# iwa-shi/CRDR

Hardware: AMD Instinct MI355X
Metric: stage-3 training img/s at 256x256 (higher is better)
Workload: dtype fp32; 1 GPU; config/crdr_stage_3.yaml -b 16: full GAN step (G + 5x CLIC21GVAE D + LPIPS-Alex, random-init weights), rate index cycled 0..4; global_batch=16, crop=256, parallelism=dp1

## Files before the change

crdr_amd/csrc/igemm.hip:

```cpp
#include <algorithm>
#include <type_traits>

#include "algo_id.hpp"
#include "igemm_kernel.hpp"
#include "wino.hpp"

namespace crdr {

extern template __global__ void igemm_kernel<4, 1, 1, 1, false, 0, false>(const IgemmArgs, const IgemmTaps, const IgemmGroup);
extern template __global__ void igemm_kernel<4, 1, 1, 2, false, 0, false>(const IgemmArgs, const IgemmTaps, const IgemmGroup);
extern template __global__ void igemm_kernel<4, 1, 1, 3, false, 0, false>(const IgemmArgs, const IgemmTaps, const IgemmGroup);
extern template __global__ void igemm_kernel<4, 1, 1, 4, false, 0, false>(const IgemmArgs, const IgemmTaps, const IgemmGroup);
extern template __global__ void igemm_kernel<4, 1, 1, 5, false, 0, false>(const IgemmArgs, const IgemmTaps, const IgemmGroup);
extern template __global__ void igemm_kernel<4, 1, 1, 6, false, 0, false>(const IgemmArgs, const IgemmTaps, const IgemmGroup);
extern template __global__ void igemm_kernel<4, 1, 1, 7, false, 0, false>(const IgemmArgs, const IgemmTaps, const IgemmGroup);
extern template __global__ void igemm_kernel<4, 1, 2, 2, false, 0, false>(const IgemmArgs, const IgemmTaps, const IgemmGroup);
extern template __global__ void igemm_kernel<4, 1, 2, 3, false, 0, false>(const IgemmArgs, const IgemmTaps, const IgemmGroup);
extern template __global__ void igemm_kernel<4, 1, 2, 4, false, 0, false>(const IgemmArgs, const IgemmTaps, const IgemmGroup);
extern template __global__ void igemm_kernel<2, 2, 2, 2, false, 0, false>(const IgemmArgs, const IgemmTaps, const IgemmGroup);
extern template __global__ void igemm_kernel<2, 2, 1, 1, false, 0, false>(const IgemmArgs, const IgemmTaps, const IgemmGroup);
extern template __global__ void igemm_kernel<2, 2, 1, 2, false, 0, false>(const IgemmArgs, const IgemmTaps, const IgemmGroup);
extern template __global__ void igemm_kernel<2, 2, 1, 3, false, 0, false>(const IgemmArgs, const IgemmTaps, const IgemmGroup);
extern template __global__ void igemm_kernel<2, 2, 1, 4, false, 0, false>(const IgemmArgs, const IgemmTaps, const IgemmGroup);
extern template __global__ void igemm_kernel<1, 4, 1, 1, false, 0, false>(const IgemmArgs, const IgemmTaps, const IgemmGroup);
extern template __global__ void igemm_kernel<1, 4, 1, 2, false, 0, false>(const IgemmArgs, const IgemmTaps, const IgemmGroup);
extern template __global__ void igemm_kernel<4, 2, 1, 1, false, 0, false>(const IgemmArgs, const IgemmTaps, const IgemmGroup);
extern template __global__ void igemm_kernel<4, 2, 1, 2, false, 0, false>(const IgemmArgs, const IgemmTaps, const IgemmGroup);
extern template __global__ void igemm_kernel<4, 2, 1, 3, false, 0, false>(const IgemmArgs, const IgemmTaps, const IgemmGroup);
extern template __global__ void igemm_kernel<4, 2, 2, 1, false, 0, false>(const IgemmArgs, const IgemmTaps, const IgemmGroup);
extern template __global__ void igemm_kernel<4, 2, 2, 2, false, 0, false>(const IgemmArgs, const IgemmTaps, const IgemmGroup);
extern template __global__ void igemm_kernel<2, 4, 1, 1, false, 0, false>(const IgemmArgs, const IgemmTaps, const IgemmGroup);
extern template __global__ void igemm_kernel<2, 4, 2, 1, false, 0, false>(const IgemmArgs, const IgemmTaps, const IgemmGroup);
extern template __global__ void igemm_kernel<2, 4, 1, 2, false, 0, false>(const IgemmArgs, const IgemmTaps, const IgemmGroup);
extern template __global__ void igemm_kernel<2, 2, 2, 1, false, 0, false>(const IgemmArgs, const IgemmTaps, const IgemmGroup);
extern template __global__ void igemm_kernel<2, 2, 2, 3, false, 0, false>(const IgemmArgs, const IgemmTaps, const IgemmGroup);
extern template __global__ void igemm_kernel<4, 1, 1, 1, true, 0, false>(const IgemmArgs, const IgemmTaps, const IgemmGroup);
extern template __global__ void igemm_kernel<4, 1, 1, 2, true, 0, false>(const IgemmArgs, const IgemmTaps, const IgemmGroup);
extern template __global__ void igemm_kernel<4, 1, 2, 2, true, 0, false>(const IgemmArgs, const IgemmTaps, const IgemmGroup);
extern template __global__ void igemm_kernel<2, 2, 2, 2, true, 0, false>(const IgemmArgs, const IgemmTaps, const IgemmGroup);
extern template __global__ void igemm_kernel<4, 2, 1, 1, true, 0, false>(const IgemmArgs, const IgemmTaps, const IgemmGroup);
extern template __global__ void igemm_kernel<4, 2, 1, 2, true, 0, false>(const IgemmArgs, const IgemmTaps, const IgemmGroup);
extern template __global__ void igemm_kernel<4, 2, 2, 1, true, 0, false>(const IgemmArgs, const IgemmTaps, const IgemmGroup);
extern template __global__ void igemm_kernel<4, 2, 2, 2, true, 0, false>(const IgemmArgs, const IgemmTaps, const IgemmGroup);
extern template __global__ void igemm_kernel<2, 4, 2, 1, true, 0, false>(const IgemmArgs, const IgemmTaps, const IgemmGroup);
extern template __global__ void igemm_kernel<4, 1, 1, 1, false, 3, false>(const IgemmArgs, const IgemmTaps, const IgemmGroup);
extern template __global__ void igemm_kernel<4, 1, 1, 2, false, 3, false>(const IgemmArgs, const IgemmTaps, const IgemmGroup);
extern template __global__ void igemm_kernel<4, 1, 1, 3, false, 3, false>(const IgemmArgs, const IgemmTaps, const IgemmGroup);
extern template __global__ void igemm_kernel<4, 1, 1, 4, false, 3, false>(const IgemmArgs, const IgemmTaps, const IgemmGroup);
extern template __global__ void igemm_kernel<4, 1, 1, 5, false, 3, false>(const IgemmArgs, const IgemmTaps, const IgemmGroup);
extern template __global__ void igemm_kernel<4, 1, 1, 6, false, 3, false>(const IgemmArgs, const IgemmTaps, const IgemmGroup);
extern template __global__ void igemm_kernel<4, 1, 1, 7, false, 3, false>(const IgemmArgs, const IgemmTaps, const IgemmGroup);
extern template __global__ void igemm_kernel<4, 1, 2, 2, false, 3, false>(const IgemmArgs, const IgemmTaps, const IgemmGroup);
extern template __global__ void igemm_kernel<4, 1, 2, 3, false, 3, false>(const IgemmArgs, const IgemmTaps, const IgemmGroup);
extern template __global__ void igemm_kernel<4, 1, 2, 4, false, 3, false>(const IgemmArgs, const IgemmTaps, const IgemmGroup);
extern template __global__ void igemm_kernel<2, 2, 2, 2, false, 3, false>(const IgemmArgs, const IgemmTaps, const IgemmGroup);
extern template __global__ void igemm_kernel<2, 2, 1, 1, false, 3, false>(const IgemmArgs, const IgemmTaps, const IgemmGroup);
extern template __global__ void igemm_kernel<2, 2, 1, 2, false, 3, false>(const IgemmArgs, const IgemmTaps, const IgemmGroup);
extern template __global__ void igemm_kernel<2, 2, 1, 3, false, 3, false>(const IgemmArgs, const IgemmTaps, const IgemmGroup);
extern template __global__ void igemm_kernel<2, 2, 1, 4, false, 3, false>(const IgemmArgs, const IgemmTaps, const IgemmGroup);
extern template __global__ void igemm_kernel<1, 4, 1, 1, false, 3, false>(const IgemmArgs, const IgemmTaps, const IgemmGroup);
extern template __global__ void igemm_kernel<1, 4, 1, 2, false, 3, false>(const IgemmArgs, const IgemmTaps, const IgemmGroup);
extern template __global__ void igemm_kernel<4, 2, 1, 1, false, 3, false>(const IgemmArgs, const IgemmTaps, const IgemmGroup);
extern template __global__ void igemm_kernel<4, 2, 1, 2, false, 3, false>(const IgemmArgs, const IgemmTaps, const IgemmGroup);
extern template __global__ void igemm_kernel<4, 2, 1, 3, false, 3, false>(const IgemmArgs, const IgemmTaps, const IgemmGroup);
extern template __global__ void igemm_kernel<4, 2, 2, 1, false, 3, false>(const IgemmArgs, const IgemmTaps, const IgemmGroup);
extern template __global__ void igemm_kernel<4, 2, 2, 2, false, 3, false>(const IgemmArgs, const IgemmTaps, const IgemmGroup);
extern template __global__ void igemm_kernel<2, 4, 1, 1, false, 3, false>(const IgemmArgs, const IgemmTaps, const IgemmGroup);
extern template __global__ void igemm_kernel<2, 4, 2, 1, false, 3, false>(const IgemmArgs, const IgemmTaps, const IgemmGroup);
extern template __global__ void igemm_kernel<2, 4, 1, 2, false, 3, false>(const IgemmArgs, const IgemmTaps, const IgemmGroup);
extern template __global__ void igemm_kernel<2, 2, 2, 1, false, 3, false>(const IgemmArgs, const IgemmTaps, const IgemmGroup);
extern template __global__ void igemm_kernel<2, 2, 2, 3, false, 3, false>(const IgemmArgs, const IgemmTaps, const IgemmGroup);
extern template __global__ void igemm_kernel<4, 1, 1, 2, false, 6, false>(const IgemmArgs, const IgemmTaps, const IgemmGroup);
extern template __global__ void igemm_kernel<4, 1, 1, 4, false, 6, false>(const IgemmArgs, const IgemmTaps, const IgemmGroup);
extern template __global__ void igemm_kernel<2, 2, 2, 2, false, 6, false>(const IgemmArgs, const IgemmTaps, const IgemmGroup);
extern template __global__ void igemm_kernel<2, 2, 1, 1, false, 6, false>(const IgemmArgs, const IgemmTaps, const IgemmGroup);
extern template __global__ void igemm_kernel<2, 2, 1, 2, false, 6, false>(const IgemmArgs, const IgemmTaps, const IgemmGroup);
extern template __global__ void igemm_kernel<2, 2, 1, 3, false, 6, false>(const IgemmArgs, const IgemmTaps, const IgemmGroup);
extern template __global__ void igemm_kernel<4, 2, 1, 2, false, 6, false>(const IgemmArgs, const IgemmTaps, const IgemmGroup);
extern template __global__ void igemm_kernel<2, 4, 2, 1, false, 6, false>(const IgemmArgs, const IgemmTaps, const IgemmGroup);
extern template __global__ void igemm_kernel<2, 2, 2, 1, false, 6, false>(const IgemmArgs, const IgemmTaps, const IgemmGroup);
extern template __global__ void igemm_kernel<4, 1, 1, 1, false, 0, true>(const IgemmArgs, const IgemmTaps, const IgemmGroup);
extern template __global__ void igemm_kernel<4, 1, 1, 2, false, 0, true>(const IgemmArgs, const IgemmTaps, const IgemmGroup);
extern template __global__ void igemm_kernel<4, 1, 1, 3, false, 0, true>(const IgemmArgs, const IgemmTaps, const IgemmGroup);
extern template __global__ void igemm_kernel<4, 1, 1, 4, false, 0, true>(const IgemmArgs, const IgemmTaps, const IgemmGroup);
extern template __global__ void igemm_kernel<4, 1, 1, 5, false, 0, true>(const IgemmArgs, const IgemmTaps, const IgemmGroup);
extern template __global__ void igemm_kernel<4, 1, 1, 6, false, 0, true>(const IgemmArgs, const IgemmTaps, const IgemmGroup);
extern template __global__ void igemm_kernel<4, 1, 1, 7, false, 0, true>(const IgemmArgs, const IgemmTaps, const IgemmGroup);
extern template __global__ void igemm_kernel<4, 1, 2, 2, false, 0, true>(const IgemmArgs, const IgemmTaps, const IgemmGroup);
extern template __global__ void igemm_kernel<4, 1, 2, 3, false, 0, true>(const IgemmArgs, const IgemmTaps, const IgemmGroup);
extern template __global__ void igemm_kernel<4, 1, 2, 4, false, 0, true>(const IgemmArgs, const IgemmTaps, const IgemmGroup);
extern template __global__ void igemm_kernel<2, 2, 2, 2, false, 0, true>(const IgemmArgs, const IgemmTaps, const IgemmGroup);
extern template __global__ void igemm_kernel<2, 2, 1, 1, false, 0, true>(const IgemmArgs, const IgemmTaps, const IgemmGroup);
extern template __global__ void igemm_kernel<2, 2, 1, 2, false, 0, true>(const IgemmArgs, const IgemmTaps, const IgemmGroup);
extern template __global__ void igemm_kernel<2, 2, 1, 3, false, 0, true>(const IgemmArgs, const IgemmTaps, const IgemmGroup);
extern template __global__ void igemm_kernel<2, 2, 1, 4, false, 0, true>(const IgemmArgs, const IgemmTaps, const IgemmGroup);
extern template __global__ void igemm_kernel<1, 4, 1, 1, false, 0, true>(const IgemmArgs, const IgemmTaps, const IgemmGroup);
extern template __global__ void igemm_kernel<1, 4, 1, 2, false, 0, true>(const IgemmArgs, const IgemmTaps, const IgemmGroup);
extern template __global__ void igemm_kernel<4, 2, 1, 1, false, 0, true>(const IgemmArgs, const IgemmTaps, const IgemmGroup);
extern template __global__ void igemm_kernel<4, 2, 1, 2, false, 0, true>(const IgemmArgs, const IgemmTaps, const IgemmGroup);
extern template __global__ void igemm_kernel<4, 2, 1, 3, false, 0, true>(const IgemmArgs, const IgemmTaps, const IgemmGroup);
extern template __global__ void igemm_kernel<4, 2, 2, 1, false, 0, true>(const IgemmArgs, const IgemmTaps, const IgemmGroup);
extern template __global__ void igemm_kernel<4, 2, 2, 2, false, 0, true>(const IgemmArgs, const IgemmTaps, const IgemmGroup);
extern template __global__ void igemm_kernel<2, 4, 1, 1, false, 0, true>(const IgemmArgs, const IgemmTaps, const IgemmGroup);
extern template __global__ void igemm_kernel<2, 4, 2, 1, false, 0, true>(const IgemmArgs, const IgemmTaps, const IgemmGroup);
extern template __global__ void igemm_kernel<2, 4, 1, 2, false, 0, true>(const IgemmArgs, const IgemmTaps, const IgemmGroup);
extern template __global__ void igemm_kernel<2, 2, 2, 1, false, 0, true>(const IgemmArgs, const IgemmTaps, const IgemmGroup);
extern template __global__ void igemm_kernel<2, 2, 2, 3, false, 0, true>(const IgemmArgs, const IgemmTaps, const IgemmGroup);

using IgemmKern = void (*)(const IgemmArgs, const IgemmTaps, const IgemmGroup);
enum TileForm {
  kPlain,
  kTapMajor,
  kBf3,
  kFast,
  kBf6,
  kNumTileForms
};
struct TileCfg {
  int wm, wn, mb, nb;
  IgemmKern kern[kNumTileForms];
};
static constexpr size_t cfg_lds(int wm, int wn, int mb, int nb, int prec) {
  const size_t BM = 32 * wm * mb, BN = 32 * wn * nb;
  const size_t staging = igemm_staging_floats((int)BM, (int)BN, prec);
  const size_t epi = (size_t)wm * wn * 32 * 32 * (nb < 4 ? nb : 4) + (size_t)wm * 2 * BN;
  const size_t sv_off = ((staging > epi ? staging : epi) + 3) & ~(size_t)3;
  return (sv_off + (size_t)4 * BN + 4) * sizeof(float);
}
template <int a, int b, int c, int d, bool FITS = igemm_bf6_ok(a, b, c, d) && (cfg_lds(a, b, c, d, 6) <= 160 * 1024)>
struct Bf6Kern { static constexpr IgemmKern fn = igemm_kernel<a, b, c, d, false, 6>; };
template <int a, int b, int c, int d>
struct Bf6Kern<a, b, c, d, false> { static constexpr IgemmKern fn = nullptr; };
#define CFG(a, b, c, d) {a, b, c, d, {igemm_kernel<a, b, c, d, false, 0>, nullptr, igemm_kernel<a, b, c, d, false, 3>, igemm_kernel<a, b, c, d, false, 0, true>, Bf6Kern<a, b, c, d>::fn}}
#define CFGS(a, b, c, d) {a, b, c, d, {igemm_kernel<a, b, c, d, false, 0>, igemm_kernel<a, b, c, d, true, 0>, igemm_kernel<a, b, c, d, false, 3>, igemm_kernel<a, b, c, d, false, 0, true>, Bf6Kern<a, b, c, d>::fn}}
static const TileCfg kCfgs[] = {
    CFGS(4, 1, 1, 1), CFGS(4, 1, 1, 2), CFG(4, 1, 1, 3), CFG(4, 1, 1, 4), CFG(4, 1, 1, 5), CFG(4, 1, 1, 6),
    CFG(4, 1, 1, 7),
    CFGS(4, 1, 2, 2), CFG(4, 1, 2, 3), CFG(4, 1, 2, 4),
    CFGS(2, 2, 2, 2),
    CFG(2, 2, 1, 1),
    CFG(2, 2, 1, 2),
    CFG(2, 2, 1, 3),
    CFG(2, 2, 1, 4),
    CFG(1, 4, 1, 1),
    CFG(1, 4, 1, 2),
    CFGS(4, 2, 1, 1),
    CFGS(4, 2, 1, 2),
    CFG(4, 2, 1, 3),
    CFGS(4, 2, 2, 1),
    CFGS(4, 2, 2, 2),
    CFG(2, 4, 1, 1),
    CFGS(2, 4, 2, 1),
    CFG(2, 4, 1, 2),
    CFG(2, 2, 2, 1),
    CFG(2, 2, 2, 3),
};
#undef CFG
#undef CFGS
static const int kNumCfgs = sizeof(kCfgs) / sizeof(kCfgs[0]);

struct Plan {
  IgemmArgs a;
  IgemmTaps t;
  int cfg;
  int stream;
  WinoKernel wino;
  StreamArgs sa;
  dim3 grid;
  size_t lds;
  size_t ws_bytes;
};

static bool splitk_ok(long long tiles, int M, int ws_ld, int ns) {
  return tiles <= CRDR_CONV_TICKETS && (long long)ns * M * ws_ld * 4 < (1ll << 31) - (1 << 24);
}

static int floordiv(int a, int b) {
  int q = a / b, r = a % b;
  return (r != 0 && ((r < 0) != (b < 0))) ? q - 1 : q;
}

static const float kCfgTflops[] = {107, 120, 122, 120, 105, 99, 94, 90, 101, 106, 102, 116, 123, 120, 107, 109, 111, 115, 126, 121,
                                   111, 116, 119, 127, 114, 119, 108};
static_assert(sizeof(kCfgTflops) / sizeof(kCfgTflops[0]) == sizeof(kCfgs) / sizeof(kCfgs[0]), "one figure per configuration");

static void fill_taps(const crdr_conv_desc* d, IgemmArgs& a, IgemmTaps& tp) {
  auto pack_tap = [](int dh, int dw, int widx) { return (dh & 0xff) | ((dw & 0xff) << 8) | (widx << 16); };
  const int S = d->stride, P = d->pad;
  int nt = 0;
  if (!d->transposed) {
    a.nphase = 1; a.GH = d->OH; a.GW = d->OW; a.so = 1; a.si = S;
    tp.poh[0] = 0; tp.pow[0] = 0; tp.tap_begin[0] = 0;
    for (int r = 0; r < d->kh; ++r)
      for (int s = 0; s < d->kw; ++s) {
        tp.packed[nt++] = pack_tap(r - P, s - P, r * d->kw + s);
      }
    tp.tap_begin[1] = (short)nt;
  } else {
    a.nphase = S * S; a.GH = cdiv(d->OH, S); a.GW = cdiv(d->OW, S); a.so = S; a.si = 1;
    int ph = 0;
    for (int py = 0; py < S; ++py)
      for (int px = 0; px < S; ++px, ++ph) {
        tp.poh[ph] = (int8_t)py; tp.pow[ph] = (int8_t)px; tp.tap_begin[ph] = (short)nt;
        for (int r = 0; r < d->kh; ++r) {
          if (((py + P - r) % S + S) % S) continue;
          for (int s = 0; s < d->kw; ++s) {
            if (((px + P - s) % S + S) % S) continue;
            tp.packed[nt++] = pack_tap(floordiv(py + P - r, S), floordiv(px + P - s, S), r * d->kw + s);
          }
        }
      }
    tp.tap_begin[ph] = (short)nt;
  }
}

static int plan_geometry(const crdr_conv_desc* d, Plan* pl, int G) {
  IgemmArgs& a = pl->a;
  IgemmTaps& tp = pl->t;
  memset(&a, 0, sizeof(a));
  memset(&tp, 0, sizeof(tp));
  CRDR_REQUIRE(d->kh * d->kw <= 128, "conv2d: kernel %dx%d has more than 128 taps", d->kh, d->kw);
  CRDR_REQUIRE(d->stride >= 1 && d->stride <= 4, "conv2d: stride %d unsupported", d->stride);
  CRDR_REQUIRE(d->C % 4 == 0 && d->ldx % 4 == 0, "conv2d: C (%d) and ldx (%d) must be multiples of 4", d->C, d->ldx);
  CRDR_REQUIRE(d->wcols % 32 == 0 && d->wcols >= d->C && d->wrows >= d->OC, "conv2d: bad weight pack %dx%d", d->wrows,
               d->wcols);
  a.N = d->N; a.H = d->H; a.W = d->W; a.Cin = d->C; a.ldx = d->ldx;
  a.OH = d->OH; a.OW = d->OW; a.ldy = d->ldy; a.Cout = d->OC;
  a.wrows = d->wrows; a.wcols = d->wcols;
  a.ldres = d->ldres; a.ldg = d->ldg; a.flags = d->flags;
  a.ldpre = d->ldpre; a.ldmask = d->ldmask; a.ngroup = G;
  CRDR_REQUIRE(G >= 1 && G <= CRDR_MAX_GROUP, "conv2d: group of %d problems (max %d)", G, CRDR_MAX_GROUP);
  a.smallc = d->wlayout == 1;
  CRDR_REQUIRE(!a.smallc || (!d->transposed && d->C <= 4 && d->wcols >= 4 * d->kh * d->kw),
               "conv2d: tap-major weight layout needs a non-transposed conv with C <= 4 and wcols >= 4*taps");
  a.kchunks = a.smallc ? cdiv(d->kh * d->kw, 8) : cdiv(d->C, 32);
  fill_taps(d, a, tp);
  {
    const long long hw = (long long)a.GH * a.GW;
    const bool p2 = a.GW > 0 && hw > 0 && hw < (1ll << 30) && (a.GW & (a.GW - 1)) == 0 && (hw & (hw - 1)) == 0;
    a.gw_sh = p2 ? __builtin_ctz((unsigned)a.GW) : -1;
    a.hw_sh = p2 ? __builtin_ctzll((unsigned long long)hw) : -1;
  }
  {
    const long long xb = (((long long)d->N * d->H * d->W - 1) * d->ldx + d->C) * 4;
    const long long wb = (long long)(a.smallc ? 1 : d->kh * d->kw) * d->wrows * d->wcols * 4;
    CRDR_REQUIRE(wb < (1ll << 31), "conv2d: weight pack (%lld B) reaches 2 GiB", wb);
    CRDR_REQUIRE((long long)d->W * d->ldx * 4 * (d->kh + 2) < (1ll << 30), "conv2d: an image row (%d px x %d floats) is too wide", d->W, d->ldx);
    a.x_bytes = (unsigned long long)xb;
    a.w_bytes = (unsigned)wb;
  }
  const long long M64 = (long long)d->N * a.GH * a.GW;
  CRDR_REQUIRE(M64 < (1ll << 31) && (long long)d->N * d->H * d->W < (1ll << 31), "conv2d: too many pixels");
  a.M = (int)M64;
  CRDR_REQUIRE(!((d->flags & CRDR_CONV_BF16X6) && (d->flags & CRDR_CONV_BF16X3)), "conv2d: CRDR_CONV_BF16X3 and CRDR_CONV_BF16X6 are exclusive");
  a.cs_ld = round_up(d->OC, 32);
  a.nsplit = 1;
  pl->cfg = pl->stream = -1;
  pl->wino = WinoKernel::None;
  pl->grid = dim3(1, 1, 1);
  pl->lds = pl->ws_bytes = 0;
  return 0;
}

static int plan_wino(const crdr_conv_desc* d, Plan* pl, int G, const AlgoId& id, bool fallback) {
  const bool f4 = id.family == kAlgoWino4;
  int nsplit = 1;
  if (f4) {
    CRDR_REQUIRE(!fallback && wino4_eligible(d, G, true), "conv2d: forced F(4x4, 3x3) Winograd kernel: not a 3x3 / 5x5 stride-1 or 5x5 stride-2 convolution it takes (wino4_eligible)");
    nsplit = conv_algo_splits(id);
    CRDR_REQUIRE(wino4_split_ok(d, G, nsplit), "conv2d: F(4x4, 3x3) Winograd kernel: %d K splits do not fit this shape", nsplit);
  } else {
    CRDR_REQUIRE(!fallback && wino_eligible(d, G), "conv2d: forced Winograd kernel: not a 3x3 / 5x5 stride-1 convolution it takes");
    CRDR_REQUIRE(id.index == 0 || wino_pairs_ok(d), "conv2d: Winograd pair-tile variant: needs a channel tail of 1..32 and more than one patch");
    CRDR_REQUIRE(id.split == 0, "conv2d: the Winograd kernel has no split-K");
  }
  pl->wino = f4 ? WinoKernel::F4 : (id.index == 1 ? WinoKernel::F2Pairs : WinoKernel::F2);
  pl->a.nsplit = nsplit;
  if (d->flags & CRDR_EPI_COLSUM) pl->a.cs_rows = f4 ? wino4_colsum_rows(d) : wino_colsum_rows(d);
  pl->ws_bytes = (size_t)CRDR_CONV_TICKETS * sizeof(int) + (f4 ? wino4_workspace(d, G, nsplit) : wino_workspace(d, G));
  return 0;
}

static int choose_stream(const crdr_conv_desc* d, const IgemmArgs& a, int G) {
  if ((d->flags & CRDR_EPI_COLSUM) || (long long)a.M * G < 16384 || d->ldy % 4 != 0 || ((d->flags & CRDR_EPI_RES) && d->ldres % 4 != 0) ||
      ((d->flags & (CRDR_EPI_RELUMASK | CRDR_EPI_LRELUMASK)) && d->ldmask % 4 != 0))
    return -1;
  static const int pref[] = {1, 2, 0, 3};
  long long bestpad = 1ll << 60;
  int best = -1;
  for (int q = 0; q < 4; ++q) {
    const int sv = 4 + pref[q];
    size_t lds;
    if (sv >= stream_num_variants() || stream_fits(d, sv, &lds) != StreamFit::kOk) continue;
    int snb, sst, snw;
    stream_variant_shape(sv, &snb, &sst, &snw);
    const long long pad = (long long)cdiv(d->OC, 32 * snb) * (32 * snb);
    if (pad < bestpad) { bestpad = pad; best = sv; }
  }
  return best;
}

static int plan_stream(const crdr_conv_desc* d, Plan* pl, int G, int sv, int forced_split) {
  IgemmArgs& a = pl->a;
  CRDR_REQUIRE(forced_split == 0, "conv2d: the streaming 1x1 kernel has no split-K");
  size_t lds = 0;
  const StreamFit fit = stream_fits(d, sv, &lds);
  CRDR_REQUIRE(fit != StreamFit::kShape,
               "conv2d: the streaming kernel takes 1x1 stride-1 convolutions with C %% 32 == 0, OC %% 4 == 0 and no "
               "gate / pre-add / accumulate epilogue");
  int snb, sstages, snw;
  stream_variant_shape(sv, &snb, &sstages, &snw);
  const int BN = 32 * snb, SBM = 32 * snw;
  CRDR_REQUIRE(fit != StreamFit::kLds, "conv2d: streaming variant %d needs %zu B of LDS for C = %d", sv, lds, d->C);
  const int gridN = cdiv(d->OC, BN), mtiles = cdiv(a.M, SBM);
  CRDR_REQUIRE(fit != StreamFit::kColumnTiles, "conv2d: streaming variant %d: %d column tiles", sv, gridN);
  const int nlanes = std::max(8, std::min(256 / (gridN * G) / 8 * 8, round_up(mtiles, 8)));
  pl->stream = sv;
  pl->sa.gridN = gridN;
  pl->sa.nlanes = nlanes;
  pl->grid = dim3(G * gridN * nlanes, 1, 1);
  pl->lds = lds;
  if (d->flags & CRDR_EPI_COLSUM) a.cs_rows = mtiles;
  return 0;
}

static void choose_tile(const crdr_conv_desc* d, const IgemmArgs& a, int KT, int G, int max_split, int* bc, int* bs) {
  double best = 1e300;
  const bool bf6 = (d->flags & CRDR_CONV_BF16X6) && !a.smallc;
  for (int c = 0; c < kNumCfgs; ++c) {
    const TileCfg& t = kCfgs[c];
    if (a.smallc && !t.kern[kTapMajor]) continue;
    if (bf6 && !t.kern[kBf6]) continue;
    const int BM = 32 * t.wm * t.mb, BN = 32 * t.wn * t.nb;
    const long long tiles = (long long)cdiv(a.M, BM) * cdiv(d->OC, BN) * a.nphase;
    for (int ns = 1; ns <= max_split; ns *= 2) {
      if (ns > 1 && KT / ns < 4) break;
      if (ns > 1 && !splitk_ok(tiles * G, a.M, cdiv(d->OC, BN) * BN, ns)) break;
      const long long blocks = tiles * ns * G;
      const double per_iter = 16.0 * t.mb * t.nb * 64.0 * std::max(1.0, t.wm * t.wn / 4.0) * (133.0 / kCfgTflops[c]) *
                              ((d->flags & CRDR_CONV_BF16X3) && !a.smallc ? 0.3 : (bf6 ? 0.5 : 1.0));
      const double waves = (double)cdiv64(blocks, 256);
      double cost = waves * ((double)cdiv(KT, ns) * per_iter + 3000.0);
      if (ns > 1) cost += 7000.0 + (double)BM * BN * ns * 4.0 / 40.0;
      if (cost < best) { best = cost; *bc = c; *bs = ns; }
    }
  }
}

static int plan_tiled(const crdr_conv_desc* d, Plan* pl, int G, const AlgoId& id, bool fallback) {
  IgemmArgs& a = pl->a;
  int maxtaps = 0;
  for (int ph = 0; ph < a.nphase; ++ph) maxtaps = std::max(maxtaps, (int)(pl->t.tap_begin[ph + 1] - pl->t.tap_begin[ph]));
  const int KT = a.smallc ? a.kchunks : maxtaps * a.kchunks;
  const bool bf6 = (d->flags & CRDR_CONV_BF16X6) && !a.smallc;
  int bc = -1, bs = 1;
  if (id.family == kAlgoBuiltIn) {
    choose_tile(d, a, KT, G, (fallback || (d->flags & CRDR_CONV_NOSPLIT)) ? 1 : 16, &bc, &bs);
  } else {
    bc = id.index;
    bs = conv_algo_splits(id);
    CRDR_REQUIRE(id.family == kAlgoTiled, "conv2d: forced config %d out of range", bc);
    CRDR_REQUIRE(!a.smallc || kCfgs[bc].kern[kTapMajor], "conv2d: config %d has no tap-major variant", bc);
    CRDR_REQUIRE(!bf6 || kCfgs[bc].kern[kBf6], "conv2d: config %d has no bf16x6 variant (its stages do not fit LDS)", bc);
    CRDR_REQUIRE(bs == 1 || KT / bs >= 2, "conv2d: forced split %d too deep for %d K-iterations", bs, KT);
    CRDR_REQUIRE(bs == 1 || !(d->flags & CRDR_CONV_NOSPLIT), "conv2d: forced split %d with CRDR_CONV_NOSPLIT", bs);
    if (bs > 1) {
      const TileCfg& ft = kCfgs[bc];
      const int fBM = 32 * ft.wm * ft.mb, fBN = 32 * ft.wn * ft.nb;
      CRDR_REQUIRE(splitk_ok((long long)cdiv(a.M, fBM) * cdiv(d->OC, fBN) * a.nphase * G, a.M, cdiv(d->OC, fBN) * fBN, bs),
                   "conv2d: forced split %d: too many tiles or slabs too large for the in-launch reduce", bs);
    }
  }
  CRDR_REQUIRE(bc >= 0, "conv2d: no tile config");
  const TileCfg& t = kCfgs[bc];
  const int BM = 32 * t.wm * t.mb, BN = 32 * t.wn * t.nb;
  pl->cfg = bc;
  a.nsplit = bs;
  pl->grid = dim3(cdiv(a.M, BM), cdiv(d->OC, BN), a.nphase * bs * G);
  {
    const double A = (double)d->N * d->H * d->W * d->C * 4.0, B = (double)a.w_bytes;
    a.m_inner = (G == 1 && B >= 32.0e6 && A * 4.0 <= B) ? 1 : 0;
  }
  a.ws_ld = pl->grid.y * BN;
  {
    static const int mode = [] { const char* e = getenv("CRDR_K_CMAJOR"); return e ? atoi(e) : -1; }();
    const bool applies = !a.smallc && maxtaps > 1 && a.kchunks > 1;
    a.k_cmajor = applies && (mode == 1 || (mode < 0 && d->C >= 1024)) ? 1 : 0;
  }
  pl->lds = cfg_lds(t.wm, t.wn, t.mb, t.nb, bf6 ? 6 : 0);
  if (d->flags & CRDR_EPI_COLSUM) a.cs_rows = a.nphase * (int)pl->grid.x;
  pl->ws_bytes = bs > 1 ? (size_t)CRDR_CONV_TICKETS * sizeof(int) + (size_t)G * a.nphase * bs * a.M * a.ws_ld * sizeof(float) : 0;
  return 0;
}

static int build_plan(const crdr_conv_desc* d, Plan* pl, int G = 1, bool fallback = false) {
  if (int rc = plan_geometry(d, pl, G)) return rc;
  const AlgoId id = conv_algo_decode(d->reserved, kNumCfgs, stream_num_variants());
  if (id.family == kAlgoWino2 || id.family == kAlgoWino4) return plan_wino(d, pl, G, id, fallback);
  int sv = id.family == kAlgoStream ? id.index : -1;
  if (id.family == kAlgoBuiltIn && !fallback) sv = choose_stream(d, pl->a, G);
  if (sv >= 0) return plan_stream(d, pl, G, sv, id.split);
  return plan_tiled(d, pl, G, id, fallback);
}

}

using namespace crdr;

extern "C" int crdr_conv2d_num_configs(void) { return kNumCfgs; }
extern "C" int crdr_conv2d_num_stream_configs(void) { return stream_num_variants(); }
extern "C" int crdr_conv2d_num_wino_configs(void) { return 3; }

extern "C" size_t crdr_conv2d_grouped_workspace(const crdr_conv_desc* d, int G) {
  Plan pl;
  return build_plan(d, &pl, G) ? 0 : pl.ws_bytes;
}
extern "C" size_t crdr_conv2d_workspace(const crdr_conv_desc* d) { return crdr_conv2d_grouped_workspace(d, 1); }

extern "C" int crdr_conv2d_colsum_layout(const crdr_conv_desc* d, int G, int* rows, int* ld) {
  CRDR_REQUIRE(d && rows && ld, "conv2d_colsum_layout: null pointer");
  Plan pl;
  if (int rc = build_plan(d, &pl, G)) return rc;
  *rows = pl.a.cs_rows;
  *ld = pl.a.cs_ld;
  return 0;
}

extern "C" int crdr_conv2d_choose_algo(const crdr_conv_desc* d, int G) {
  Plan pl;
  if (!d || build_plan(d, &pl, G)) return 0;
  const bool f4 = pl.wino == WinoKernel::F4, f2 = pl.wino == WinoKernel::F2 || pl.wino == WinoKernel::F2Pairs;
  const AlgoFamily family = f4 ? kAlgoWino4 : (f2 ? kAlgoWino2 : (pl.stream >= 0 ? kAlgoStream : kAlgoTiled));
  const int index = f4 ? 0 : (f2 ? (pl.wino == WinoKernel::F2Pairs ? 1 : 0) : (pl.stream >= 0 ? pl.stream : pl.cfg));
  return conv_algo_encode(family, index, pl.a.nsplit, kNumCfgs, stream_num_variants());
}

extern "C" double crdr_conv2d_flops(const crdr_conv_desc* d) {
  if (!d->transposed) return 2.0 * d->N * d->OH * d->OW * (double)d->OC * d->C * d->kh * d->kw;
  return 2.0 * d->N * d->H * d->W * (double)d->OC * d->C * d->kh * d->kw;
}

static bool al16(const void* q) { return (reinterpret_cast<uintptr_t>(q) & 15) == 0; }

static int check_io(const crdr_conv_desc* d, const crdr_conv_io* ios, int G, size_t need_ws, size_t ws_bytes) {
  const crdr_conv_io& io = ios[0];
  const int flags = d->flags;
  CRDR_REQUIRE(!(flags & CRDR_EPI_VEC2) || io.vec2, "conv2d: VEC2 flag without vec2");
  CRDR_REQUIRE(!(flags & CRDR_EPI_RES) || io.res, "conv2d: RES flag without res");
  CRDR_REQUIRE(!((flags & CRDR_EPI_RELUMASK) && (flags & CRDR_EPI_LRELUMASK)), "conv2d: RELUMASK and LRELUMASK are exclusive");
  CRDR_REQUIRE(!(flags & CRDR_EPI_AFFINE) || (io.scale && io.shift), "conv2d: AFFINE flag without scale/shift");
  CRDR_REQUIRE(!(flags & CRDR_EPI_GATE) || (io.gx && io.gt && io.sig), "conv2d: GATE flag without gx/gt/sig");
  CRDR_REQUIRE(G == 1 || !(flags & (CRDR_EPI_VEC2 | CRDR_EPI_AFFINE | CRDR_EPI_GATE | CRDR_EPI_MASKOFF)),
               "conv2d_grouped: epilogue flags %d not supported in a grouped launch", flags);
  CRDR_REQUIRE(!(flags & CRDR_EPI_MASKOFF) || ((flags & (CRDR_EPI_RELUMASK | CRDR_EPI_LRELUMASK)) && io.vec2 && !(flags & CRDR_EPI_VEC2)),
               "conv2d: MASKOFF needs a mask flag and vec2, and excludes VEC2");
  CRDR_REQUIRE(need_ws <= ws_bytes, "conv2d: workspace too small (%zu < %zu)", ws_bytes, need_ws);
  for (int g = 0; g < G; ++g) {
    const crdr_conv_io& q = ios[g];
    CRDR_REQUIRE(q.x && q.w && q.y, "conv2d: null tensor (problem %d)", g);
    CRDR_REQUIRE(al16(q.x) && al16(q.w), "conv2d: x and w must be 16-byte aligned (problem %d)", g);
    CRDR_REQUIRE(!(flags & CRDR_EPI_BIAS) || q.bias, "conv2d: BIAS flag without bias (problem %d)", g);
    CRDR_REQUIRE(!(flags & CRDR_EPI_PREADD) || q.pre, "conv2d: PREADD flag without pre (problem %d)", g);
    CRDR_REQUIRE(!(flags & (CRDR_EPI_RELUMASK | CRDR_EPI_LRELUMASK)) || q.mask, "conv2d: mask flag without mask (problem %d)", g);
    CRDR_REQUIRE(!(flags & CRDR_EPI_RES) || q.res, "conv2d: RES flag without res (problem %d)", g);
    CRDR_REQUIRE(!(flags & CRDR_EPI_COLSUM) || q.cs, "conv2d: COLSUM flag without cs (problem %d)", g);
  }
  return 0;
}

static bool rows_aligned(const crdr_conv_desc* d, const crdr_conv_io* ios, int G) {
  const bool res = d->flags & CRDR_EPI_RES, gate = d->flags & CRDR_EPI_GATE, pre = d->flags & CRDR_EPI_PREADD;
  const bool mask = d->flags & (CRDR_EPI_RELUMASK | CRDR_EPI_LRELUMASK);
  bool v = d->ldy % 4 == 0 && (!res || d->ldres % 4 == 0) && (!pre || d->ldpre % 4 == 0) && (!mask || d->ldmask % 4 == 0) &&
           (!gate || (d->ldg % 4 == 0 && al16(ios[0].gx) && al16(ios[0].gt) && al16(ios[0].sig)));
  for (int g = 0; g < G; ++g) {
    const crdr_conv_io& q = ios[g];
    v = v && al16(q.y) && (!res || al16(q.res)) && (!pre || al16(q.pre)) && (!mask || al16(q.mask));
  }
  return v;
}

static bool fast_epilogue_ok(const IgemmArgs& a, bool vec_epi) {
  const long long span_px = (256 / std::max(a.GW, 1) + 2) * (long long)std::max(a.so, 1) * a.OW + a.OW;
  const long long span = span_px * std::max(std::max(a.ldy, a.ldres), a.ldmask) * 4;
  return vec_epi && a.Cout % 4 == 0 && span < (1ll << 31) && !(a.flags & (CRDR_EPI_GATE | CRDR_EPI_PREADD | CRDR_EPI_ACCUM));
}

static void bind_io(Plan* pl, const crdr_conv_io* ios, int G, void* ws, IgemmGroup* grp) {
  IgemmArgs& a = pl->a;
  const crdr_conv_io& io = ios[0];
  a.x = io.x; a.w = io.w; a.y = io.y;
  a.counters = (int*)ws;
  a.ws = (float*)ws + CRDR_CONV_TICKETS;
  a.bias = io.bias; a.vec2 = io.vec2; a.res = io.res; a.scale = io.scale; a.shift = io.shift;
  a.gx = io.gx; a.gt = io.gt; a.sig = io.sig; a.pre = io.pre; a.mask = io.mask; a.cs = io.cs;
  memset(grp, 0, sizeof(*grp));
  for (int g = 0; g < G; ++g) {
    const crdr_conv_io& q = ios[g];
    grp->x[g] = q.x; grp->w[g] = q.w; grp->y[g] = q.y; grp->bias[g] = q.bias; grp->pre[g] = q.pre; grp->mask[g] = q.mask;
    grp->res[g] = q.res; grp->cs[g] = q.cs;
  }
}

static int launch_conv(const crdr_conv_desc* d, const crdr_conv_io* ios, int G, void* ws, size_t ws_bytes, crdr_stream_t s,
                       float* ucache = nullptr, size_t ucache_bytes = 0, int ucache_valid = 0) {
  Plan pl;
  if (int rc = build_plan(d, &pl, G)) return rc;
  if (pl.a.M == 0) return 0;
  if (int rc = check_io(d, ios, G, pl.ws_bytes, ws_bytes)) return rc;
  const bool vec_epi = rows_aligned(d, ios, G);
  if (pl.stream >= 0 && !vec_epi && d->reserved == 0) {
    if (int rc = build_plan(d, &pl, G, true)) return rc;
  }
  IgemmGroup grp;
  bind_io(&pl, ios, G, ws, &grp);
  IgemmArgs& a = pl.a;
  a.vec_epi = vec_epi ? 1 : 0;
  a.fast_epi = fast_epilogue_ok(a, vec_epi) ? 1 : 0;
  if (pl.wino != WinoKernel::None) {
    const bool f4 = pl.wino == WinoKernel::F4;
    void* prof = profile_begin(as_stream(s));
    if (f4) {
      const size_t u_bytes = wino4_workspace(d, G, 1);
      float* u = (float*)ws + CRDR_CONV_TICKETS;
      if (ucache) {
        CRDR_REQUIRE(ucache_bytes >= u_bytes, "conv2d: filter cache of %zu bytes, the launch needs %zu", ucache_bytes, u_bytes);
        u = ucache;
      }
      float* slabs = (float*)ws + CRDR_CONV_TICKETS + u_bytes / 4;
      if (int rc = wino4_launch(d, a, pl.t, grp, G, u, slabs, a.nsplit, ucache && ucache_valid, as_stream(s))) return rc;
    } else if (int rc = wino_launch(d, pl.wino == WinoKernel::F2Pairs, a, pl.t, grp, G, (float*)ws + CRDR_CONV_TICKETS, as_stream(s))) return rc;
    profile_end(f4 ? (d->kh == 5 ? 6 : 5) : 3, G * crdr_conv2d_flops(d), prof, as_stream(s));
    return 0;
  }
  if (pl.stream >= 0) {
    CRDR_REQUIRE(a.vec_epi, "conv2d: the streaming kernel needs 16-byte aligned operand rows");
    void* prof = profile_begin(as_stream(s));
    stream_launch(pl.stream, a, pl.sa, grp, pl.grid.x, pl.lds, as_stream(s));
    CRDR_CHECK_LAUNCH("gemm1x1_kernel");
    profile_end(0, G * crdr_conv2d_flops(d), prof, as_stream(s));
    return 0;
  }
  const TileCfg& t = kCfgs[pl.cfg];
  const TileForm form = a.smallc ? kTapMajor : ((d->flags & CRDR_CONV_BF16X3) ? kBf3 : ((d->flags & CRDR_CONV_BF16X6) ? kBf6 : ((a.fast_epi && a.nsplit == 1) ? kFast : kPlain)));
  const IgemmKern kern = t.kern[form];
  CRDR_REQUIRE(kern, "conv2d: config %d has no kernel for this precision", pl.cfg);
  static std::atomic<bool> attr_done[kNumTileForms][64];
  allow_full_lds(attr_done[form][pl.cfg], kern);
  void* prof = profile_begin(as_stream(s));
  hipLaunchKernelGGL(kern, pl.grid, dim3(64 * t.wm * t.wn), pl.lds, as_stream(s), a, pl.t, grp);
  CRDR_CHECK_LAUNCH("igemm_kernel");
  profile_end(0, G * crdr_conv2d_flops(d), prof, as_stream(s));
  return 0;
}

extern "C" int crdr_conv2d(const crdr_conv_desc* d, const crdr_conv_io* io, void* ws, size_t ws_bytes,
                           crdr_stream_t s) {
  CRDR_REQUIRE(d && io, "conv2d: null descriptor");
  return launch_conv(d, io, 1, ws, ws_bytes, s);
}

extern "C" int crdr_conv2d_grouped(const crdr_conv_desc* d, const crdr_conv_io* ios, int G, void* ws, size_t ws_bytes,
                                   crdr_stream_t s) {
  CRDR_REQUIRE(d && ios, "conv2d_grouped: null descriptor");
  CRDR_REQUIRE(G >= 1 && G <= CRDR_MAX_GROUP, "conv2d_grouped: %d problems (1..%d)", G, CRDR_MAX_GROUP);
  return launch_conv(d, ios, G, ws, ws_bytes, s);
}

extern "C" size_t crdr_conv2d_filter_cache_bytes(const crdr_conv_desc* d, int G) {
  Plan pl;
  if (!d || G < 1 || G > CRDR_MAX_GROUP || build_plan(d, &pl, G) || pl.wino != WinoKernel::F4) return 0;
  return wino4_workspace(d, G, 1);
}

extern "C" int crdr_conv2d_filter_item(const crdr_conv_desc* d, int G, crdr_w4_filter_item* item) {
  CRDR_REQUIRE(d && item, "conv2d_filter_item: null pointer");
  CRDR_REQUIRE(G >= 1 && G <= CRDR_MAX_GROUP, "conv2d_filter_item: %d problems (1..%d)", G, CRDR_MAX_GROUP);
  Plan pl;
  if (int rc = build_plan(d, &pl, G)) return rc;
  CRDR_REQUIRE(pl.wino == WinoKernel::F4, "conv2d_filter_item: the descriptor's `reserved` does not force the F(4x4, 3x3) kernel");
  return wino4_filter_item(d, pl.t, G, item);
}

extern "C" int crdr_w4_filters_batched(const crdr_w4_filter_item* items, const int64_t* prefix, const int64_t* meta, crdr_stream_t s) {
  CRDR_REQUIRE(items && prefix && meta, "w4_filters_batched: null pointer");
  return wino4_filters_batched(items, reinterpret_cast<const long long*>(prefix), reinterpret_cast<const long long*>(meta), as_stream(s));
}

extern "C" int crdr_conv2d_grouped_ex(const crdr_conv_desc* d, const crdr_conv_io* ios, int G, void* ws, size_t ws_bytes, float* filter_cache,
                                      size_t filter_cache_bytes, int filter_cache_valid, crdr_stream_t s) {
  CRDR_REQUIRE(d && ios, "conv2d_grouped_ex: null descriptor");
  CRDR_REQUIRE(G >= 1 && G <= CRDR_MAX_GROUP, "conv2d_grouped_ex: %d problems (1..%d)", G, CRDR_MAX_GROUP);
  CRDR_REQUIRE(!filter_cache || (reinterpret_cast<uintptr_t>(filter_cache) & 15) == 0, "conv2d_grouped_ex: the filter cache must be 16-byte aligned");
  return launch_conv(d, ios, G, ws, ws_bytes, s, filter_cache, filter_cache_bytes, filter_cache_valid);
}
```

crdr_amd/csrc/igemm_args.hpp:

```cpp
#pragma once

#include "common.hpp"

namespace crdr {

struct IgemmArgs {
  const float* x;
  const float* w;
  float* y;
  float* ws;
  const float* bias;
  const float* vec2;
  const float* res;
  const float* scale;
  const float* shift;
  const float* gx;
  const float* gt;
  float* sig;
  const float* pre;
  const float* mask;
  int* counters;
  float* cs;
  int ldpre, ldmask;
  int cs_ld, cs_rows;
  int ngroup;
  int N, H, W, Cin, ldx;
  int GH, GW, so, OH, OW, ldy, Cout;
  int si;
  int wrows, wcols;
  int ldres, ldg;
  int flags;
  int M;
  int nphase, nsplit;
  int kchunks;
  int ws_ld;
  int hw_sh, gw_sh;
  int vec_epi;
  int m_inner;
  int fast_epi;
  int k_cmajor;
  int smallc;
  unsigned long long x_bytes;
  unsigned w_bytes;
};

struct IgemmTaps {
  int packed[128];
  short tap_begin[17];
  int8_t poh[16], pow[16];
};

struct IgemmGroup {
  const float* x[CRDR_MAX_GROUP];
  const float* w[CRDR_MAX_GROUP];
  float* y[CRDR_MAX_GROUP];
  const float* bias[CRDR_MAX_GROUP];
  const float* pre[CRDR_MAX_GROUP];
  const float* mask[CRDR_MAX_GROUP];
  const float* res[CRDR_MAX_GROUP];
  float* cs[CRDR_MAX_GROUP];
};

typedef __attribute__((address_space(3))) void* lds_ptr_t;
static constexpr unsigned kOobOffset = 0x80000000u;

struct StreamArgs {
  int gridN;
  int nlanes;
};
int stream_num_variants();
void stream_variant_shape(int v, int* nb, int* stages, int* nw);
enum class StreamFit { kOk, kShape, kLds, kColumnTiles };
StreamFit stream_fits(const crdr_conv_desc* d, int v, size_t* lds);
void stream_launch(int v, const IgemmArgs& a, const StreamArgs& sa, const IgemmGroup& grp, unsigned grid, size_t lds, hipStream_t s);

}
```

Baseline: 224.7 img/s.

## Add persistent streaming MFMA kernel for 4-channel RGB input convolutions

Adds a dedicated persistent kernel for convolutions whose input has only 4 channels (padded RGB) with 3x3 or 5x5 kernels at stride 1 or 2. Each wave keeps its 64-column weight slice in registers, prefetches the next pixel strip into registers while computing the current one, and applies the fused epilogue through LDS. The aim is to replace the generic tap-major implicit-GEMM path, which wastes work on these narrow-K first layers. It adds a new code path with its own LDS budget and bounds handling, and can be turned off with CRDR_RGBCONV=0.

```diff
diff --git a/crdr_amd/csrc/igemm.hip b/crdr_amd/csrc/igemm.hip
--- a/crdr_amd/csrc/igemm.hip
+++ b/crdr_amd/csrc/igemm.hip
@@ -541,6 +541,12 @@
     profile_end(0, G * crdr_conv2d_flops(d), prof, as_stream(s));
     return 0;
   }
+  if (rgbconv_eligible(d, a, G)) {
+    void* prof = profile_begin(as_stream(s));
+    if (int rc = rgbconv_launch(d, a, as_stream(s))) return rc;
+    profile_end(0, G * crdr_conv2d_flops(d), prof, as_stream(s));
+    return 0;
+  }
   const TileCfg& t = kCfgs[pl.cfg];
   const TileForm form = a.smallc ? kTapMajor : ((d->flags & CRDR_CONV_BF16X3) ? kBf3 : ((d->flags & CRDR_CONV_BF16X6) ? kBf6 : ((a.fast_epi && a.nsplit == 1) ? kFast : kPlain)));
   const IgemmKern kern = t.kern[form];
diff --git a/crdr_amd/csrc/igemm_args.hpp b/crdr_amd/csrc/igemm_args.hpp
--- a/crdr_amd/csrc/igemm_args.hpp
+++ b/crdr_amd/csrc/igemm_args.hpp
@@ -74,4 +74,7 @@
 StreamFit stream_fits(const crdr_conv_desc* d, int v, size_t* lds);
 void stream_launch(int v, const IgemmArgs& a, const StreamArgs& sa, const IgemmGroup& grp, unsigned grid, size_t lds, hipStream_t s);
 
+bool rgbconv_eligible(const crdr_conv_desc* d, const IgemmArgs& a, int G);
+int rgbconv_launch(const crdr_conv_desc* d, const IgemmArgs& a, hipStream_t s);
+
 }
diff --git a/crdr_amd/csrc/rgbconv.hip b/crdr_amd/csrc/rgbconv.hip
--- /dev/null
+++ b/crdr_amd/csrc/rgbconv.hip
@@ -0,0 +1,242 @@
+#include <stdlib.h>
+
+#include <algorithm>
+#include <type_traits>
+
+#include "igemm_args.hpp"
+
+namespace crdr {
+
+struct RgbConvArgs {
+  const float* x;
+  const float* w;
+  float* y;
+  const float* bias;
+  const float* vec2;
+  const float* scale;
+  const float* shift;
+  int N, H, W, ldx;
+  int OH, OW, ldy, Cout;
+  int wrows, wcols;
+  int pad, flags;
+  int nslice;
+  int nwave;
+  int spr;
+  int nstrip;
+};
+
+static constexpr int kRgbSliceCols = 64;
+static constexpr int kRgbStripPx = 32;
+static constexpr int rgb_waves_per_simd(int k, int s) { return (k <= 3 && s == 1) ? 4 : 2; }
+static constexpr int rgb_in_floats(int k, int s) { return ((k * ((kRgbStripPx - 1) * s + k) * 4) + 3) & ~3; }
+static constexpr int rgb_wave_floats(int k, int s) { return rgb_in_floats(k, s) + kRgbStripPx * 32 + 4 * kRgbSliceCols; }
+
+template <int K, int S>
+__global__ __launch_bounds__(256, rgb_waves_per_simd(K, S)) void rgbconv_kernel(const RgbConvArgs p) {
+  constexpr int T = K * K, NP = (T + 1) / 2;
+  constexpr int WD = (kRgbStripPx - 1) * S + K;
+  constexpr int NPIECE = K * WD, NLD = (NPIECE + 63) / 64;
+  constexpr int CLD = kRgbSliceCols;
+  extern __shared__ __attribute__((aligned(16))) float smem[];
+  const int tid = threadIdx.x, lane = tid & 63, wave = __builtin_amdgcn_readfirstlane(tid >> 6);
+  float* sIn = smem + wave * rgb_wave_floats(K, S);
+  float* sC = sIn + rgb_in_floats(K, S);
+  float* sV = sC + kRgbStripPx * 32;
+  const int gw = blockIdx.x * 4 + wave;
+  const int slice = gw % p.nslice, worker = gw / p.nslice;
+  const int nworker = (p.nwave - slice + p.nslice - 1) / p.nslice;
+  const int n0 = slice * kRgbSliceCols;
+  const int frow = lane & 31, fh = lane >> 5;
+
+  constexpr int CH = K <= 3 ? NP : 4, WLD = CH * 8 + 4;
+  static_assert(32 * WLD <= rgb_wave_floats(K, S), "the weight staging must fit the wave's LDS");
+  f32x4 bf[NP][2];
+  bool lane3 = false;
+#pragma unroll
+  for (int j = 0; j < 2; ++j)
+#pragma unroll
+    for (int c0 = 0; c0 < NP; c0 += CH) {
+      constexpr int NPC = 32 * CH * 2;
+#pragma unroll
+      for (int i = 0; i < (NPC + 63) / 64; ++i) {
+        const int idx = lane + 64 * i, row = idx / (CH * 2), pc = idx % (CH * 2);
+        const int oc = n0 + 32 * j + row, tap = 2 * c0 + pc;
+        f32x4 v = {0.f, 0.f, 0.f, 0.f};
+        if (idx < NPC && oc < p.wrows && tap < T) v = *reinterpret_cast<const f32x4*>(p.w + (size_t)oc * p.wcols + tap * 4);
+        if (idx < NPC) *reinterpret_cast<f32x4*>(sIn + row * WLD + pc * 4) = v;
+      }
+#pragma unroll
+      for (int tp = c0; tp < c0 + CH && tp < NP; ++tp) {
+        const f32x4 v = *reinterpret_cast<const f32x4*>(sIn + frow * WLD + ((tp - c0) * 2 + fh) * 4);
+        bf[tp][j] = v;
+        const float w3 = v[3];
+        lane3 = lane3 || (__builtin_bit_cast(unsigned, w3) << 1) != 0u;
+      }
+    }
+  const int f = p.flags;
+  {
+    const bool live = n0 + lane < p.Cout;
+    sV[0 * CLD + lane] = (live && (f & CRDR_EPI_BIAS)) ? p.bias[n0 + lane] : 0.f;
+    sV[1 * CLD + lane] = (live && (f & CRDR_EPI_VEC2)) ? p.vec2[n0 + lane] : 0.f;
+    sV[2 * CLD + lane] = (live && (f & CRDR_EPI_AFFINE)) ? p.scale[n0 + lane] : 1.f;
+    sV[3 * CLD + lane] = (live && (f & CRDR_EPI_AFFINE)) ? p.shift[n0 + lane] : 0.f;
+  }
+  const float* fa = sIn + frow * S * 4;
+
+  f32x4 stage[NLD];
+  auto request = [&](int sidx) __attribute__((always_inline)) {
+    const int owb = sidx % p.spr, t = sidx / p.spr;
+    const int oh = t % p.OH, n = t / p.OH;
+    const int ih0 = oh * S - p.pad, iw0 = owb * (kRgbStripPx * S) - p.pad;
+    const float* img = p.x + (size_t)n * p.H * p.W * p.ldx;
+#pragma unroll
+    for (int i = 0; i < NLD; ++i) {
+      const int idx = lane + 64 * i;
+      const int ih = idx < NPIECE ? ih0 + idx / WD : -1, iw = iw0 + idx % WD;
+      f32x4 v = {0.f, 0.f, 0.f, 0.f};
+      if ((unsigned)ih < (unsigned)p.H && (unsigned)iw < (unsigned)p.W) v = *reinterpret_cast<const f32x4*>(img + ((size_t)ih * p.W + iw) * p.ldx);
+      stage[i] = v;
+    }
+  };
+
+  auto walk = [&](auto nch) __attribute__((always_inline)) {
+    constexpr int NCH = decltype(nch)::value;
+    int sidx = worker;
+    if (sidx < p.nstrip) request(sidx);
+    for (; sidx < p.nstrip; sidx += nworker) {
+#pragma unroll
+      for (int i = 0; i < NLD; ++i)
+        if (lane + 64 * i < NPIECE) *reinterpret_cast<f32x4*>(sIn + (lane + 64 * i) * 4) = stage[i];
+      const int owb = sidx % p.spr, t = sidx / p.spr;
+      if (sidx + nworker < p.nstrip) request(sidx + nworker);
+
+      f32x16 acc[2];
+#pragma unroll
+      for (int j = 0; j < 2; ++j)
+#pragma unroll
+        for (int r = 0; r < 16; ++r) acc[j][r] = 0.f;
+#pragma unroll
+      for (int tp = 0; tp < NP; ++tp) {
+        const int t0 = 2 * tp, t1 = (2 * tp + 1 < T) ? 2 * tp + 1 : 2 * tp;
+        const int o0 = ((t0 / K) * WD + t0 % K) * 4, o1 = ((t1 / K) * WD + t1 % K) * 4;
+        f32x4 af = *reinterpret_cast<const f32x4*>(fa + (fh ? o1 : o0));
+        if (2 * tp + 1 >= T && fh) af = f32x4{0.f, 0.f, 0.f, 0.f};
+#pragma unroll
+        for (int s = 0; s < NCH; ++s)
+#pragma unroll
+          for (int j = 0; j < 2; ++j) acc[j] = __builtin_amdgcn_mfma_f32_32x32x2f32(af[s], bf[tp][j][s], acc[j], 0, 0, 0);
+      }
+
+      const int ow0 = owb * kRgbStripPx;
+      const int c4 = lane & 7, prow = lane >> 3;
+#pragma unroll
+      for (int j = 0; j < 2; ++j) {
+#pragma unroll
+        for (int r = 0; r < 16; ++r) sC[((r & 3) + 8 * (r >> 2) + 4 * fh) * 32 + frow] = acc[j][r];
+        const int cc = j * 32 + c4 * 4;
+        f32x4 o[4];
+#pragma unroll
+        for (int kq = 0; kq < 4; ++kq) o[kq] = *reinterpret_cast<const f32x4*>(sC + (prow + 8 * kq) * 32 + c4 * 4);
+        if (f & CRDR_EPI_BIAS) {
+#pragma unroll
+          for (int kq = 0; kq < 4; ++kq) o[kq] += *reinterpret_cast<const f32x4*>(sV + 0 * CLD + cc);
+        }
+        if (f & CRDR_EPI_RELU) {
+#pragma unroll
+          for (int kq = 0; kq < 4; ++kq)
+#pragma unroll
+            for (int e = 0; e < 4; ++e) o[kq][e] = fmaxf(o[kq][e], 0.0f);
+        }
+        if (f & CRDR_EPI_LRELU) {
+#pragma unroll
+          for (int kq = 0; kq < 4; ++kq)
+#pragma unroll
+            for (int e = 0; e < 4; ++e) o[kq][e] = o[kq][e] > 0.0f ? o[kq][e] : 0.2f * o[kq][e];
+        }
+        if (f & CRDR_EPI_VEC2) {
+#pragma unroll
+          for (int kq = 0; kq < 4; ++kq) o[kq] += *reinterpret_cast<const f32x4*>(sV + 1 * CLD + cc);
+        }
+        if (f & CRDR_EPI_AFFINE) {
+          const f32x4 vscale = *reinterpret_cast<const f32x4*>(sV + 2 * CLD + cc), vshift = *reinterpret_cast<const f32x4*>(sV + 3 * CLD + cc);
+#pragma unroll
+          for (int kq = 0; kq < 4; ++kq)
+#pragma unroll
+            for (int e = 0; e < 4; ++e) o[kq][e] = o[kq][e] * vscale[e] + vshift[e];
+        }
+        float* yrow = p.y + ((size_t)t * p.OW + ow0) * p.ldy + n0 + cc;
+#pragma unroll
+        for (int kq = 0; kq < 4; ++kq) {
+          const int row = prow + 8 * kq;
+          if (n0 + cc < p.Cout && ow0 + row < p.OW) *reinterpret_cast<f32x4*>(yrow + (size_t)row * p.ldy) = o[kq];
+        }
+      }
+    }
+  };
+  if (__builtin_amdgcn_ballot_w64(lane3) != 0)
+    walk(std::integral_constant<int, 4>{});
+  else
+    walk(std::integral_constant<int, 3>{});
+}
+
+using RgbKern = void (*)(const RgbConvArgs);
+struct RgbVariant {
+  int k, s;
+  RgbKern kern;
+  size_t wave_bytes;
+};
+#define RGBV(k, s) {k, s, rgbconv_kernel<k, s>, sizeof(float) * rgb_wave_floats(k, s)}
+static const RgbVariant kRgbVariants[] = {RGBV(3, 1), RGBV(3, 2), RGBV(5, 1), RGBV(5, 2)};
+#undef RGBV
+
+static const RgbVariant* rgb_variant(const crdr_conv_desc* d) {
+  if (d->kh != d->kw) return nullptr;
+  for (const RgbVariant& v : kRgbVariants)
+    if (v.k == d->kh && v.s == d->stride) return &v;
+  return nullptr;
+}
+
+static bool rgbconv_enabled() {
+  static const bool on = [] { const char* e = getenv("CRDR_RGBCONV"); return !(e && e[0] == '0'); }();
+  return on;
+}
+
+bool rgbconv_eligible(const crdr_conv_desc* d, const IgemmArgs& a, int G) {
+  const int epi = CRDR_EPI_BIAS | CRDR_EPI_RELU | CRDR_EPI_LRELU | CRDR_EPI_VEC2 | CRDR_EPI_AFFINE;
+  const int ignored = CRDR_CONV_BF16X3 | CRDR_CONV_BF16X6 | CRDR_CONV_NOSPLIT;
+  if (!rgbconv_enabled() || !a.smallc || G != 1 || d->transposed || a.nsplit != 1 || !a.fast_epi) return false;
+  if (d->flags & ~(epi | ignored)) return false;
+  if (d->C != 4 || d->ldx % 4 != 0 || d->OC % 4 != 0 || d->ldy % 4 != 0) return false;
+  if (d->OC > 4 * kRgbSliceCols) return false;
+  return rgb_variant(d) != nullptr;
+}
+
+int rgbconv_launch(const crdr_conv_desc* d, const IgemmArgs& a, hipStream_t s) {
+  const RgbVariant* v = rgb_variant(d);
+  CRDR_REQUIRE(v, "conv2d: the streaming RGB kernel has no %dx%d stride-%d variant", d->kh, d->kw, d->stride);
+  RgbConvArgs p;
+  p.x = a.x; p.w = a.w; p.y = a.y; p.bias = a.bias; p.vec2 = a.vec2; p.scale = a.scale; p.shift = a.shift;
+  p.N = d->N; p.H = d->H; p.W = d->W; p.ldx = d->ldx;
+  p.OH = d->OH; p.OW = d->OW; p.ldy = d->ldy; p.Cout = d->OC;
+  p.wrows = d->wrows; p.wcols = d->wcols;
+  p.pad = d->pad; p.flags = d->flags;
+  p.nslice = cdiv(d->OC, kRgbSliceCols);
+  p.spr = cdiv(d->OW, kRgbStripPx);
+  const long long nstrip = (long long)d->N * d->OH * p.spr;
+  CRDR_REQUIRE(nstrip < (1ll << 31), "conv2d: too many pixel strips");
+  p.nstrip = (int)nstrip;
+  const int wgs_per_cu = rgb_waves_per_simd(v->k, v->s);
+  const int grid = (int)std::max(1ll, std::min((long long)wgs_per_cu * cu_count(), (long long)cdiv64(nstrip * p.nslice, 4)));
+  p.nwave = grid * 4;
+  const size_t lds = v->wave_bytes * 4;
+  CRDR_REQUIRE(lds * wgs_per_cu <= 160 * 1024, "conv2d: the streaming RGB kernel needs %zu B of LDS per workgroup", lds);
+  static std::atomic<bool> attr_done;
+  RgbKern kerns[sizeof(kRgbVariants) / sizeof(kRgbVariants[0])];
+  for (size_t i = 0; i < sizeof(kRgbVariants) / sizeof(kRgbVariants[0]); ++i) kerns[i] = kRgbVariants[i].kern;
+  allow_full_lds(attr_done, kerns, (int)(sizeof(kRgbVariants) / sizeof(kRgbVariants[0])));
+  hipLaunchKernelGGL(v->kern, dim3(grid), dim3(256), lds, s, p);
+  CRDR_CHECK_LAUNCH("rgbconv_kernel");
+  return 0;
+}
+
+}
```

Result: no change. 226.0 img/s (median of 6 runs) (+0.6%).
